# jimmc414/semantic_merge

Hardware: AMD Instinct MI355X
Metric: op-log compose+conflict throughput (ops/s), 100M-op logs, 1/2/4/8 GPUs (higher is better)
Workload: dtype u64; 1 GPU; c3: one merge of 100,000,000 ops (100,000,000 per GPU), 1,000,000 symbols, 64 ops/ms, seed 11; n_ops_per_gpu=100000000, n_ops_total=100000000, n_sym=1000000, composed_ops=99989720, conflicts=5140, plan=presorted, parallelism=single GPU

## Files before the change

semantic_merge_amd/csrc/smx_compose.hip:

```cpp
#include <algorithm>
#include <atomic>
#include <cstring>
#include <mutex>
#include <string>
#include <vector>

#include "smx_sort.h"
#include "smx_window.h"
#include "smx_small.h"
#include "smx_tables.h"


#include "smx_prof.h"

#include "smx_plan.h"
#include "smx_walk.h"

#include "smx_emit.h"


struct Layout {
  size_t off[64];
  size_t total;
};
// ... 341 lines not shown
      *out = g_side[i];
      return SMX_OK;
    }
  if (g_nside == SIDE_MAX) return SMX_OK;
  SideStream* S = new SideStream;
  S->dev = dev;
  S->caller = caller;
  int ncu = 0;
  HIP_TRY(hipDeviceGetAttribute(&ncu, hipDeviceAttributeMultiprocessorCount, dev));
  const int k = knob("SMX_SIDE_CUS", 0);
  if (k > 0 && k < ncu) {
    std::vector<uint32_t> mask((size_t)(ncu + 31) / 32, 0u);
    for (int i = 0; i < k; ++i) mask[(size_t)i / 32] |= 1u << (i % 32);
    HIP_TRY(hipExtStreamCreateWithCUMask(&S->s, (uint32_t)mask.size(), mask.data()));
  } else {
    HIP_TRY(hipStreamCreateWithFlags(&S->s, hipStreamNonBlocking));
  }
  const unsigned evf = hipEventDisableTiming | hipEventDisableSystemFence;
  HIP_TRY(hipEventCreateWithFlags(&S->fork, evf));
  HIP_TRY(hipEventCreateWithFlags(&S->join, evf));
  g_side[g_nside++] = S;
  *out = S;
  return SMX_OK;
}

#ifndef SMX_TB_UNSKIP_MAXN
#define SMX_TB_UNSKIP_MAXN (1 << 22)
#endif
#ifndef SMX_TB_OVERLAP_MIN
#define SMX_TB_OVERLAP_MIN (1 << 18)
#endif

static int launch_tail(const Ctx& C) {
  u64 width, nbk;
  const bool geo = tb_geometry(C, &width, &nbk);
  SideStream* S = nullptr;
  if (geo && C.n >= SMX_TB_OVERLAP_MIN && !knob("SMX_TB_SERIAL", 0)) {
    int rc = side_stream(C.st, &S);
    if (rc) return rc;
  }
  std::unique_lock<std::mutex> own;
  int rc;
  hipStream_t st = C.st;
  TbArgs A{};
  u32* lst = C.ws<u32>(B_TBHIST);
  u32* rec = C.ws<u32>(B_REC);
  if (S) {
    own = std::unique_lock<std::mutex>(S->mu);
    A = tb_args(C);
    A.width = (u32)width;
    A.nbk = (u32)nbk;
    A.keep_skip = C.n <= SMX_TB_UNSKIP_MAXN ? 2u : 1u;
    const int nblk = (int)SMX_CEIL_DIV((u64)C.n, (u64)TB_TILE);
    HIP_TRY(hipEventRecord(S->fork, st));
    HIP_TRY(hipStreamWaitEvent(S->s, S->fork, 0));
    hipLaunchKernelGGL(k_tb_scatter, dim3(nblk), dim3(TB_NT), 0, S->s, A, lst, rec);
    HIP_TRY(hipGetLastError());
    HIP_TRY(hipEventRecord(S->join, S->s));
  }
  C.tm->begin(ST_WALK);
  if ((rc = launch_walk(C, nullptr))) {
    if (S) (void)hipStreamWaitEvent(st, S->join, 0);
    return rc;
  }
  C.tm->end(ST_WALK);
  if (S) HIP_TRY(hipStreamWaitEvent(st, S->join, 0));
  C.tm->begin(ST_TABLES);
  bool bucketed = true;
  if (S) {
    if (A.keep_skip == 1u)
      hipLaunchKernelGGL(k_tb_unskip, dim3(1024), dim3(BLOCK), 0, st, A, lst, rec, C.ws<u32>(B_SKIPLIST));
    hipLaunchKernelGGL(k_tb_reduce, dim3(nbk), dim3(TBR_NT), 0, st, A, lst, rec, C.n_sym, C.ws<int4>(B_FIN),
                       PartTab{nullptr, 0u, 0, nullptr});
    HIP_TRY(hipGetLastError());
  } else if ((rc = launch_tables(C, nullptr, 0, 0, &bucketed))) {
    return rc;
  }
  C.tm->end(ST_TABLES);
  C.tm->begin(ST_EMIT);
  if ((rc = launch_emit(C, bucketed, nullptr))) return rc;
  C.tm->end(ST_EMIT);
  return SMX_OK;
}


struct EarlyFail {
  u32* flag_host = nullptr;
  u32* flag_dev = nullptr;
  hipEvent_t ev = nullptr;
};
enum WinLevel { WL_NORMAL, WL_WIDE };
static i64 level_cap(int lv) { return lv == WL_WIDE ? WF_WIDE_CAP : WF_CAP; }
static int first_level(const Ctx& C) { return knob("SMX_FIRST_WIDE", 0) ? WL_WIDE : WL_NORMAL; }
static i64 first_tgt(const Ctx& C) {
  return knob("SMX_WIN_TGT", first_level(C) == WL_WIDE ? WF_WIDE_CAP : WIN_TGT);
}

template <int CAP, int NT, bool DBG, bool MAP>
static void launch_window_f(const WinArgs& P, hipStream_t st) {
  hipLaunchKernelGGL((k_window_f<CAP, NT, DBG, MAP>), dim3(P.W), dim3(NT), 0, st, P);
}
template <int CAP, int NT>
static void launch_window_level(const WinArgs& P, hipStream_t st) {
  if (P.src_map) launch_window_f<CAP, NT, false, true>(P, st);
  else launch_window_f<CAP, NT, false, false>(P, st);
}

static int launch_presorted_windows(const Ctx& C, i64 W, i64 CM, int level) {
  const bool wide = level == WL_WIDE;
  hipStream_t st = C.st;
  WinArgs P = win_args(C);
  P.cpre = C.ws<u32>(B_CCNT);
  P.CM = CM;
  P.kts = C.ops->ts;
  P.khi = C.ops->oid_hi;
  P.klo = C.ops->oid_lo;
  P.perm = nullptr;
  P.W = W;
  P.ablate = knob("SMX_ABLATE", 0);
  const int stage = wide ? ST_WINDOW_WIDE : ST_WINDOW;
  C.tm->begin(stage);
#if SMX_DIAG
  if (g_phase_dbg && !P.src_map && (size_t)W * WF_NSTAMP * 8 <= g_phase_dbg_bytes) {
    P.dbg = (u64*)g_phase_dbg;
    if (wide) launch_window_f<WF_WIDE_CAP, WF_WIDE_NT, true, false>(P, st);
    else launch_window_f<WF_CAP, WF_NT, true, false>(P, st);
  } else
#endif
  if (wide) launch_window_level<WF_WIDE_CAP, WF_WIDE_NT>(P, st);
  else launch_window_level<WF_CAP, WF_NT>(P, st);
  HIP_TRY(hipGetLastError());
  C.tm->end(stage);
  return SMX_OK;
}

struct Deferred {
  bool on = false;
  i64 W = 0, W_w = 0, CM = 0;
};

struct PreGeo {
  i64 tgt, W, D, CM;
  u64 *sA, *sB;
};
static PreGeo presorted_geometry(const Ctx& C, i64 tgt, int level) {
  const i64 cap = level_cap(level);
  tgt = std::min(std::max(tgt, (i64)WIN_TGT_MIN), cap);
  tgt -= tgt % CH;
  u64* sA = C.ws<u64>(B_SMP);
  return PreGeo{tgt, SMX_CEIL_DIV(C.n, tgt), cap / CH, SMX_CEIL_DIV(std::max(C.na, C.nb), (i64)CH) + 1, sA,
                sA + SMX_CEIL_DIV(C.na, (i64)CH) + 1};
}

static int run_presorted(const Ctx& C, i64 tgt, const EarlyFail* early = nullptr, int level = WL_NORMAL,
                         Deferred* defer = nullptr) {
  hipStream_t st = C.st;
  ComposeMeta* meta = C.ws<ComposeMeta>(B_META);
  i64* bnd = C.ws<i64>(B_BND);
  C.tm->begin(ST_PLAN);
  static_assert(sizeof(ComposeMeta) % 4 == 0, "meta is zeroed by words");
  const PreGeo G = presorted_geometry(C, tgt, level);
  const i64 W = G.W, CM = G.CM;
  const bool cs_small = CM <= CS_SMALL_CM;
  {
    const int rc = zero_async(meta, sizeof(ComposeMeta), st);
    if (rc) return rc;
  }
  const i64 nchunk = SMX_CEIL_DIV(C.na, (i64)CH) + SMX_CEIL_DIV(C.nb, (i64)CH);
  u32* ccnt = C.ws<u32>(B_CCNT);
  const bool lmode = early && defer && level == WL_NORMAL;
  LongW lw{};
  if (lmode) {
    const PreGeo Gw = presorted_geometry(C, level_cap(WL_WIDE), WL_WIDE);
    lw.tgt_w = Gw.tgt;
    lw.W_w = Gw.W;
    lw.D_w = Gw.D;
  }
  hipLaunchKernelGGL(k_khist, dim3(SMX_CEIL_DIV(nchunk, (i64)CH_PER_BLOCK * KH_R)), dim3(KH_NT), 0, st,
                     C.ops->kind, C.ops->ts, C.na, C.nb, C.ops->b_gap, CM, ccnt, G.sA, G.sB, meta,
                     early ? early->flag_dev : nullptr, lmode ? G.D : (i64)0);
  if (lmode) HIP_TRY(hipEventRecord(early->ev, st));
  const i64 nfp = SMX_CEIL_DIV(W + 1, (i64)BLOCK);
  const bool fused = cs_small && !early;
  if (fused)
    hipLaunchKernelGGL(k_fpart_cscan, dim3(nfp + 2 * SMX_N_KINDS), dim3(BLOCK), 0, st, C.ops->ts,
                       C.ops->ts + C.na + C.ops->b_gap, G.sA, G.sB, C.na, C.nb, W, G.tgt, G.D, bnd, meta,
                       (u32*)nullptr, ccnt, CM, nfp);
  else
    hipLaunchKernelGGL(k_fpart, dim3(nfp), dim3(BLOCK), 0, st, C.ops->ts, C.ops->ts + C.na + C.ops->b_gap, G.sA,
                       G.sB, C.na, C.nb, W, G.tgt, G.D, bnd, meta, (early && !lmode) ? early->flag_dev : nullptr, lw);
  if (early && !lmode) HIP_TRY(hipEventRecord(early->ev, st));
  const u64 nwin_long = lmode ? (u64)lw.W_w : 0ull;
  if (fused) {
  } else if (cs_small) {
    hipLaunchKernelGGL(k_cscan_small, dim3(2 * SMX_N_KINDS), dim3(BLOCK), 0, st, ccnt, C.na, C.nb, CM, meta, (u64)W,
                       nwin_long);
  } else {
    const i64 NT = SMX_CEIL_DIV(CM, (i64)CS_TILE);
    u32* tsum = C.ws<u32>(B_TSUM);
    hipLaunchKernelGGL(k_cscan_up, dim3(NT, 2 * SMX_N_KINDS), dim3(BLOCK), 0, st, ccnt, C.na, C.nb, CM, NT, tsum,
                       meta);
    hipLaunchKernelGGL(k_cscan_mid, dim3(2 * SMX_N_KINDS), dim3(BLOCK), 0, st, tsum, C.na, C.nb, CM, NT, ccnt,
                       meta, (u64)W, nwin_long);
    hipLaunchKernelGGL(k_cscan_down, dim3(NT, 2 * SMX_N_KINDS), dim3(BLOCK), 0, st, ccnt, C.na, C.nb, CM, NT,
                       tsum, meta);
  }
  HIP_TRY(hipGetLastError());
  C.tm->end(ST_PLAN);
  if (lmode) {
    *defer = Deferred{true, W, lw.W_w, CM};
    return SMX_OK;
  }
  return launch_presorted_windows(C, W, CM, level);
}

__global__ void k_plan_rearm(ComposeMeta* meta, u64 nwin) {
  if (meta->f_fail == F_LONG) meta->f_fail = 0;
  meta->n_win = nwin;
}
static int run_presorted_rewide(const Ctx& C, i64 tgt, int level = WL_WIDE) {
  hipStream_t st = C.st;
  ComposeMeta* meta = C.ws<ComposeMeta>(B_META);
  const PreGeo G = presorted_geometry(C, tgt, level);
  C.tm->begin(ST_PLAN);
  hipLaunchKernelGGL(k_plan_rearm, dim3(1), dim3(1), 0, st, meta, (u64)G.W);
  hipLaunchKernelGGL(k_fpart, dim3(SMX_CEIL_DIV(G.W + 1, (i64)BLOCK)), dim3(BLOCK), 0, st, C.ops->ts,
                     C.ops->ts + C.na + C.ops->b_gap, G.sA, G.sB, C.na, C.nb, G.W, G.tgt, G.D, C.ws<i64>(B_BND), meta,
                     (u32*)nullptr, LongW{});
  HIP_TRY(hipGetLastError());
  C.tm->end(ST_PLAN);
  return launch_presorted_windows(C, G.W, G.CM, level);
}

#include "smx_segsort.h"

static hipError_t stream_wait(hipStream_t st) { return hipStreamSynchronize(st); }

static int run_generic(const Ctx& C, int mode) {
  hipStream_t st = C.st;
  ComposeMeta* meta = C.ws<ComposeMeta>(B_META);
  i64* bnd = C.ws<i64>(B_BND);
  u32* wcnt = C.ws<u32>(B_WCNT);
  u32* woff = C.ws<u32>(B_WOFF);
  const i64 na = C.na, nb = C.nb, n = C.n;
  u64* sts = C.ws<u64>(B_STS);
  u64* shi = C.ws<u64>(B_SHI);
  u64* slo = C.ws<u64>(B_SLO);
  u32* perm = C.ws<u32>(B_PERM);
  C.tm->begin(ST_GSORT);
  HIP_TRY(hipMemsetAsync(meta, 0, sizeof(ComposeMeta), st));
  if (mode == GEN_SEG) {
    C.tm->begin(ST_SEGSORT);
    for (int side = 0; side < 2; ++side) {
      const i64 off = side ? na : 0, cnt = side ? nb : na;
      if (cnt == 0) continue;
      hipLaunchKernelGGL(k_segsort, dim3(SMX_CEIL_DIV(cnt, (i64)SEG_H)), dim3(SEG_NT), 0, st, C.ops->ts + off,
                         C.ops->oid_hi + off, C.ops->oid_lo + off, cnt, (u32)off, sts + off, shi + off, slo + off,
                         perm + off, meta);
    }
    C.tm->end(ST_SEGSORT);
  } else {
    const bool with_lo = mode == GEN_RADIX_LO;
    hipLaunchKernelGGL(k_meta_init, dim3(1), dim3(1), 0, st, meta);
    hipLaunchKernelGGL(k_keymask, dim3(grid_for(n, BLOCK * 8)), dim3(BLOCK), 0, st, C.ops->ts, C.ops->oid_hi,
                       C.ops->oid_lo, na, n, meta);
    ComposeMeta hm;
    HIP_TRY(hipMemcpyAsync(&hm, meta, sizeof(ComposeMeta), hipMemcpyDeviceToHost, st));
    HIP_TRY(hipStreamSynchronize(st));
    RadixTemp rt{C.ws<u64>(B_RK2), C.ws<u32>(B_RV2), C.ws<u32>(B_RHIST), C.ws<u32>(B_PART)};
    const u64* words[3] = {C.ops->oid_lo, C.ops->oid_hi, C.ops->ts};
    const int w0 = with_lo ? 0 : 1;
    for (int side = 0; side < 2; ++side) {
      const i64 off = side ? na : 0, cnt = side ? nb : na;
      if (cnt == 0) continue;
      u64* key = C.ws<u64>(B_RKEY) + off;
      u32* val = perm + off;
      for (int wi = w0; wi < 3; ++wi) {
        const int q = 2 - wi;
        const u64 varying = hm.key_or[side][q] ^ hm.key_and[side][q];
        int shifts[8], ns = 0;
        for (int dgt = 0; dgt < 8; ++dgt)
          if ((varying >> (8 * dgt)) & 0xffull) shifts[ns++] = 8 * dgt;
        if (wi == w0) {
          hipLaunchKernelGGL(k_gather_init, dim3(grid_for(cnt)), dim3(BLOCK), 0, st, words[wi] + off, key, val,
                             cnt);
          if (off)
            hipLaunchKernelGGL(k_offset, dim3(grid_for(cnt)), dim3(BLOCK), 0, st, val, cnt, (u32)off);
        } else {
          hipLaunchKernelGGL(k_gather, dim3(grid_for(cnt)), dim3(BLOCK), 0, st, words[wi], val, key, cnt);
        }
        if (ns) HIP_TRY(radix_sort_pairs(key, val, cnt, shifts, ns, rt, st));
      }
      HIP_TRY(hipMemcpyAsync(sts + off, key, (size_t)cnt * 8, hipMemcpyDeviceToDevice, st));
      hipLaunchKernelGGL(k_gather2, dim3(grid_for(cnt)), dim3(BLOCK), 0, st, C.ops->oid_hi, C.ops->oid_lo, val,
                         shi + off, slo + off, cnt);
    }
    if (!with_lo) hipLaunchKernelGGL(k_dupcheck, dim3(grid_for(n)), dim3(BLOCK), 0, st, sts, shi, na, n, meta);
  }
  const i64 W = SMX_CEIL_DIV(n, (i64)WG_CAP);
  hipLaunchKernelGGL(k_gpart, dim3(SMX_CEIL_DIV(W + 1, (i64)BLOCK)), dim3(BLOCK), 0, st, sts, shi, slo, na, nb,
                     W, bnd, meta);
  hipLaunchKernelGGL(k_wcount, dim3(W), dim3(WC_NT), 0, st, C.ops->kind, C.ops->v0, C.ops->v1, perm, bnd, na, W,
                     wcnt, meta);
  hipLaunchKernelGGL(k_wscan, dim3(NCNT), dim3(BLOCK), 0, st, wcnt, woff, W, meta);
  hipLaunchKernelGGL(k_bases, dim3(1), dim3(1), 0, st, meta, (u64)W);
  HIP_TRY(hipGetLastError());
  C.tm->end(ST_GSORT);
  WinArgs P = win_args(C);
  P.kts = sts;
  P.khi = shi;
  P.klo = slo;
  P.perm = perm;
  P.W = W;
  P.ablate = 0;
  C.tm->begin(ST_WINDOW_G);
  hipLaunchKernelGGL(k_window_g, dim3(W), dim3(WG_NT), 0, st, P);
  HIP_TRY(hipGetLastError());
  C.tm->end(ST_WINDOW_G);
  return SMX_OK;
}

struct PinnedMeta {
  ComposeMeta* p = nullptr;
  ~PinnedMeta() {
    if (p) (void)hipHostFree(p);
  }
};
static int read_meta(const Ctx& C, ComposeMeta* hm) {
  static thread_local PinnedMeta holder;
  ComposeMeta*& pinned = holder.p;
  if (!pinned) HIP_TRY(hipHostMalloc((void**)&pinned, sizeof(ComposeMeta), hipHostMallocDefault));
  HIP_TRY(hipMemcpyAsync(pinned, C.ws<ComposeMeta>(B_META), sizeof(ComposeMeta), hipMemcpyDeviceToHost, C.st));
// ... 386 lines not shown
```

semantic_merge_amd/csrc/smx_plan.h:

```cpp
#pragma once

__global__ void __launch_bounds__(BLOCK) k_keymask(const u64* __restrict__ ts, const u64* __restrict__ hi,
                                                   const u64* __restrict__ lo, i64 na, i64 n,
                                                   ComposeMeta* meta) {
  u64 ro[2][3] = {{0, 0, 0}, {0, 0, 0}};
  u64 ra[2][3] = {{~0ull, ~0ull, ~0ull}, {~0ull, ~0ull, ~0ull}};
  for (i64 i = (i64)blockIdx.x * BLOCK + threadIdx.x; i < n; i += (i64)gridDim.x * BLOCK) {
    const u64 v[3] = {ts[i], hi[i], lo[i]};
    const int s = i >= na;
#pragma unroll
    for (int q = 0; q < 3; ++q) {
      ro[s][q] |= v[q];
      ra[s][q] &= v[q];
    }
  }
  __shared__ u32 sm[24];
  if (threadIdx.x < 24) sm[threadIdx.x] = 0;
  __syncthreads();
#pragma unroll
  for (int s = 0; s < 2; ++s)
#pragma unroll
    for (int q = 0; q < 3; ++q) {
      const u64 w[2] = {ro[s][q], ~ra[s][q]};
#pragma unroll
// ... 2 lines not shown
        if ((threadIdx.x & (WAVE - 1)) == WAVE - 1) {
          atomicOr(&sm[(s * 3 + q) * 4 + 2 * x], lo32);
          atomicOr(&sm[(s * 3 + q) * 4 + 2 * x + 1], hi32);
        }
      }
    }
  __syncthreads();
  if (threadIdx.x < 6) {
    const int s = threadIdx.x / 3, q = threadIdx.x % 3;
    const u32* v = &sm[threadIdx.x * 4];
    atomicOr((unsigned long long*)&meta->key_or[s][q], ((unsigned long long)v[1] << 32) | v[0]);
    atomicAnd((unsigned long long*)&meta->key_and[s][q], ~(((unsigned long long)v[3] << 32) | v[2]));
  }
}

__global__ void k_zero(u32* __restrict__ p, u64 nw) {
  for (u64 i = (u64)blockIdx.x * blockDim.x + threadIdx.x; i < nw; i += (u64)gridDim.x * blockDim.x) p[i] = 0u;
}
static int zero_async(void* p, size_t bytes, hipStream_t st) {
  if (bytes % 4) return set_err(SMX_E_ARG, "zero_async: size not a multiple of 4");
  const u64 nw = bytes / 4;
  if (nw == 0) return SMX_OK;
  u64 g = SMX_CEIL_DIV(nw, (u64)BLOCK * 4);
  if (g > 4096) g = 4096;
  hipLaunchKernelGGL(k_zero, dim3((u32)g), dim3(BLOCK), 0, st, (u32*)p, nw);
  HIP_TRY(hipGetLastError());
  return SMX_OK;
}

__global__ void k_meta_init(ComposeMeta* meta) {
  for (int s = 0; s < 2; ++s)
    for (int q = 0; q < 3; ++q) meta->key_and[s][q] = ~0ull;
}

struct LongW {
  i64 tgt_w = 0, W_w = 0, D_w = 0;
};
__device__ __forceinline__ void fpart_body(const u64* __restrict__ ts, const u64* __restrict__ tsB,
                                           const u64* __restrict__ sA, const u64* __restrict__ sB, i64 na, i64 nb,
                                           i64 W, i64 tgt, i64 D, i64* __restrict__ bnd, ComposeMeta* meta,
                                           u32* long_host, i64 blk, i64 nblk, LongW lw = LongW{}) {
  const i64 k = blk * BLOCK + threadIdx.x;
  bool chk = true;
  u64 fl = F_LONG;
  if (lw.tgt_w) {
    if ((__hip_atomic_load(&meta->f_fail, __ATOMIC_RELAXED, __HIP_MEMORY_SCOPE_AGENT) & F_LONG) == F_LONG) {
      W = lw.W_w, tgt = lw.tgt_w, D = lw.D_w;
      fl = F_WLONG;
      long_host = nullptr;
    } else {
      chk = false;
    }
  }
  if (chk) {
    const i64 nt = nblk * BLOCK, ca = SMX_CEIL_DIV(na, (i64)CH), cb = nb / CH;
    bool lg = false;
    for (i64 c = k; c + D < ca; c += nt) lg |= sA[c] == sA[c + D];
    for (i64 c = k; c + D < cb; c += nt) lg |= sB[c] == sB[c + D];
    const u64 lgw = __ballot(lg);
    if (lgw && (threadIdx.x & (WAVE - 1)) == 0 &&
        (__hip_atomic_load(&meta->f_fail, __ATOMIC_RELAXED, __HIP_MEMORY_SCOPE_AGENT) & fl) != fl) {
      atomicOr((unsigned long long*)&meta->f_fail, fl);
      if (long_host) __hip_atomic_store(long_host, 1u, __ATOMIC_RELAXED, __HIP_MEMORY_SCOPE_SYSTEM);
    }
    if (lgw) {
      if (k <= W) bnd[2 * k] = bnd[2 * k + 1] = 0;
      return;
    }
  }
  if (k > W) return;
  const i64 n = na + nb;
  const u64* A = ts;
  const u64* B = tsB;
  const i64 d = k * tgt;
  if (k == 0 || d >= n || k == W) {
    bnd[2 * k] = k == 0 ? 0 : na;
    bnd[2 * k + 1] = k == 0 ? 0 : nb;
    return;
  }
  const i64 lo0 = d - nb > 0 ? d - nb : 0, hi0 = d < na ? d : na;
  i64 lo = lo0, hi = hi0;
  if (lo < hi) {
    const i64 ilo = SMX_CEIL_DIV(lo, (i64)CH), ihi = (hi - 1) / CH;
    if (ilo <= ihi) {
      const i64 dj = d / CH - 1;
      i64 l = ilo, h = ihi + 1;
      while (l < h) {
        const i64 mid = (l + h) >> 1;
        if (sA[mid] <= sB[dj - mid]) l = mid + 1;
        else h = mid;
      }
      if (l > ilo) lo = CH * (l - 1) + 1;
      if (l <= ihi) hi = CH * l;
    }
    while (lo < hi) {
      const i64 mid = (lo + hi) >> 1;
      if (A[mid] <= B[d - 1 - mid]) lo = mid + 1;
      else hi = mid;
    }
  }
  const i64 a = lo, b = d - lo;
  const u64 tau = (a < na && (b >= nb || A[a] <= B[b])) ? A[a] : B[b];
  i64 r[2];
#pragma unroll
  for (int s = 0; s < 2; ++s) {
    const u64* X = s ? B : A;
    i64 h = s ? b : a;
    i64 step = 1, l = 0;
    while (h > 0) {
      const i64 cand = h - step > 0 ? h - step : 0;
      if (X[cand] < tau) {
        l = cand + 1;
        break;
      }
      h = cand;
      step *= 2;
    }
    while (l < h) {
      const i64 mid = (l + h) >> 1;
      if (X[mid] < tau) l = mid + 1;
      else h = mid;
    }
    r[s] = l;
  }
  bnd[2 * k] = r[0];
  bnd[2 * k + 1] = r[1];
}
__global__ void k_fpart(const u64* __restrict__ ts, const u64* __restrict__ tsB, const u64* __restrict__ sA,
                        const u64* __restrict__ sB, i64 na, i64 nb, i64 W, i64 tgt, i64 D, i64* __restrict__ bnd,
                        ComposeMeta* meta, u32* long_host, LongW lw) {
  fpart_body(ts, tsB, sA, sB, na, nb, W, tgt, D, bnd, meta, long_host, blockIdx.x, gridDim.x, lw);
}

__global__ void k_gpart(const u64* __restrict__ sts, const u64* __restrict__ shi,
                        const u64* __restrict__ slo, i64 na, i64 nb, i64 W, i64* __restrict__ bnd,
                        const ComposeMeta* meta) {
  const i64 k = (i64)blockIdx.x * BLOCK + threadIdx.x;
  if (k > W || meta->f_fail) return;
  const i64 n = na + nb;
  const i64 d = k * WG_CAP;
  if (k == 0) { bnd[0] = 0; bnd[1] = 0; return; }
  if (d >= n || k == W) { bnd[2 * k] = na; bnd[2 * k + 1] = nb; return; }
  i64 lo = d - nb > 0 ? d - nb : 0, hi = d < na ? d : na;
  while (lo < hi) {
    i64 mid = (lo + hi) >> 1;
    const i64 j = na + d - 1 - mid;
    if (key_le(sts[mid], shi[mid], slo[mid], sts[j], shi[j], slo[j])) lo = mid + 1;
    else hi = mid;
  }
  bnd[2 * k] = lo;
  bnd[2 * k + 1] = d - lo;
}

#ifndef KH_NT
#define KH_NT 512
#endif
#define CH_PER_BLOCK (KH_NT / 16)
#ifndef KH_R
#define KH_R 1
#endif

__global__ void __launch_bounds__(KH_NT) k_khist(const u8* __restrict__ kind, const u64* __restrict__ ts,
                                                 i64 na, i64 nb, i64 bgap, i64 CM, u32* __restrict__ cnt,
                                                 u64* __restrict__ sA, u64* __restrict__ sB, ComposeMeta* meta,
                                                 u32* long_host, i64 Dl) {
  __shared__ u32 c[CH_PER_BLOCK * KH_R][SMX_N_KINDS];
  __shared__ u32 km[2];
  __shared__ u32 lgb;
  const i64 CA = SMX_CEIL_DIV(na, (i64)CH), CB = SMX_CEIL_DIV(nb, (i64)CH);
  const int j = threadIdx.x / 16, q = threadIdx.x % 16;
  if (threadIdx.x < 2) km[threadIdx.x] = 0;
  if (threadIdx.x == 0) lgb = 0;
  u32 w[KH_R][4];
  int nvr[KH_R];
  u64 smpA[KH_R], smpB[KH_R], farA[KH_R], farB[KH_R];
  u64* atA[KH_R];
  u64* atB[KH_R];
  bool chkA[KH_R], chkB[KH_R];
#pragma unroll
  for (int rd = 0; rd < KH_R; ++rd) {
    const i64 g = ((i64)blockIdx.x * KH_R + rd) * CH_PER_BLOCK + j;
    const int side = g >= CA;
    const i64 cc = side ? g - CA : g;
    const i64 len = side ? nb : na;
    const i64 r0 = cc * CH + q * 16;
    const int nv = g < CA + CB ? (int)(len - r0 < 0 ? 0 : (len - r0 < 16 ? len - r0 : 16)) : 0;
    nvr[rd] = nv;
    const u8* src = kind + (side ? na + bgap : 0) + r0;
    w[rd][0] = w[rd][1] = w[rd][2] = w[rd][3] = 0u;
    if (nv == 16 && (reinterpret_cast<uintptr_t>(src) & 15) == 0) {
      const uint4 v = *reinterpret_cast<const uint4*>(src);
      w[rd][0] = v.x; w[rd][1] = v.y; w[rd][2] = v.z; w[rd][3] = v.w;
    } else {
#pragma unroll
      for (int y = 0; y < 16; ++y)
        if (y < nv) w[rd][y >> 2] |= (u32)src[y] << (8 * (y & 3));
    }
    atA[rd] = atB[rd] = nullptr;
    smpA[rd] = smpB[rd] = farA[rd] = farB[rd] = 0;
    chkA[rd] = chkB[rd] = false;
    if (g < CA + CB) {
      if (!side && q == 0) {
        atA[rd] = sA + cc;
        smpA[rd] = ts[cc * CH];
        if (Dl > 0 && cc + Dl < CA) {
          chkA[rd] = true;
          farA[rd] = ts[(cc + Dl) * CH];
        }
      }
      if (side && q == 15 && nv == 16) {
        atB[rd] = sB + cc;
        smpB[rd] = ts[na + bgap + cc * CH + CH - 1];
        if (Dl > 0 && cc + Dl < nb / CH) {
          chkB[rd] = true;
          farB[rd] = ts[na + bgap + (cc + Dl) * CH + CH - 1];
        }
      }
    }
  }
  bool bad = false;
#pragma unroll
  for (int rd = 0; rd < KH_R; ++rd) {
    const int nv = nvr[rd];
    u32 pk[3] = {0u, 0u, 0u};
#pragma unroll
    for (int y = 0; y < 16; ++y) {
      if (y >= nv) break;
      u32 k = (w[rd][y >> 2] >> (8 * (y & 3))) & 0xffu;
      bad |= k >= SMX_N_KINDS;
      k = k < SMX_N_KINDS ? k : SMX_N_KINDS - 1;
      const u32 wd = (k * 43u) >> 8;
      const u32 inc = 1u << (5u * (k - 6u * wd));
      pk[0] += wd == 0 ? inc : 0u;
      pk[1] += wd == 1 ? inc : 0u;
      pk[2] += wd == 2 ? inc : 0u;
    }
    u32 f[6];
#pragma unroll
    for (int i = 0; i < 3; ++i) {
      f[2 * i] = (pk[i] & 31u) | ((pk[i] >> 5) & 31u) << 10 | ((pk[i] >> 10) & 31u) << 20;
      f[2 * i + 1] = ((pk[i] >> 15) & 31u) | ((pk[i] >> 20) & 31u) << 10 | ((pk[i] >> 25) & 31u) << 20;
    }
#pragma unroll
    for (int i = 0; i < 6; ++i) {
      u32 v = f[i];
      v += dpp_u32<0x111, 0xf>(v);
      v += dpp_u32<0x112, 0xf>(v);
      v += dpp_u32<0x114, 0xf>(v);
      v += dpp_u32<0x118, 0xf>(v);
      f[i] = v;
    }
    if (q == 15) {
#pragma unroll
      for (int k = 0; k < SMX_N_KINDS; ++k) c[rd * CH_PER_BLOCK + j][k] = (f[k / 3] >> (10 * (k % 3))) & 1023u;
    }
  }
  bool lg = false;
#pragma unroll
  for (int rd = 0; rd < KH_R; ++rd) {
    if (atA[rd]) *atA[rd] = smpA[rd];
    if (atB[rd]) *atB[rd] = smpB[rd];
    lg |= (chkA[rd] && farA[rd] == smpA[rd]) || (chkB[rd] && farB[rd] == smpB[rd]);
  }
  if (__ballot(lg) && (threadIdx.x & (WAVE - 1)) == 0) atomicOr(&lgb, 1u);
  if (__ballot(bad) && (threadIdx.x & (WAVE - 1)) == 0) {
    meta->bad_sym = 1;
    if (long_host) __hip_atomic_store(long_host + 1, 1u, __ATOMIC_RELAXED, __HIP_MEMORY_SCOPE_SYSTEM);
  }
  __syncthreads();
  if (threadIdx.x == 0 && lgb &&
      (__hip_atomic_load(&meta->f_fail, __ATOMIC_RELAXED, __HIP_MEMORY_SCOPE_AGENT) & F_LONG) != F_LONG) {
    const u64 was = atomicOr((unsigned long long*)&meta->f_fail, F_LONG);
    if ((was & F_LONG) != F_LONG && long_host)
      __hip_atomic_store(long_host, 1u, __ATOMIC_RELAXED, __HIP_MEMORY_SCOPE_SYSTEM);
  }
  u32 m0 = 0, m1 = 0;
  for (int i = threadIdx.x; i < CH_PER_BLOCK * KH_R * SMX_N_KINDS; i += KH_NT) {
    const int jj = i % (CH_PER_BLOCK * KH_R), k = i / (CH_PER_BLOCK * KH_R);
    const i64 gg = (i64)blockIdx.x * CH_PER_BLOCK * KH_R + jj;
    if (gg >= CA + CB) continue;
    const int sd = gg >= CA;
    const u32 v = c[jj][k];
    cnt[((i64)sd * SMX_N_KINDS + k) * CM + (sd ? gg - CA : gg)] = v;
    if (v) (sd ? m1 : m0) |= 1u << k;
  }
  m0 = wave_or_to_last(m0);
  m1 = wave_or_to_last(m1);
  if ((threadIdx.x & (WAVE - 1)) == WAVE - 1) {
    if (m0) atomicOr(&km[0], m0);
    if (m1) atomicOr(&km[1], m1);
  }
  __syncthreads();
  if (threadIdx.x < 2 && km[threadIdx.x]) {
    const u32 cur = __hip_atomic_load(&meta->kmask[threadIdx.x], __ATOMIC_RELAXED, __HIP_MEMORY_SCOPE_AGENT);
    if ((cur | km[threadIdx.x]) != cur) atomicOr(&meta->kmask[threadIdx.x], km[threadIdx.x]);
  }
}

__device__ __forceinline__ bool cs_present(const ComposeMeta* meta, int col) {
  return (meta->kmask[col >= SMX_N_KINDS] >> (col % SMX_N_KINDS)) & 1u;
}

#define CS_TILE (BLOCK * 8)

__global__ void __launch_bounds__(BLOCK) k_cscan_up(const u32* __restrict__ cnt, i64 na, i64 nb, i64 CM,
                                                    i64 NT, u32* __restrict__ tsum, const ComposeMeta* meta) {
  __shared__ u32 s[NWAVES + 1];
  const int col = blockIdx.y;
  if (!cs_present(meta, col)) return;
  const i64 C = SMX_CEIL_DIV(col >= SMX_N_KINDS ? nb : na, (i64)CH);
  const i64 t0 = (i64)blockIdx.x * CS_TILE;
  if (t0 >= C) return;
  const u32* colp = cnt + (i64)col * CM;
  const i64 b = t0 + (i64)threadIdx.x * 8;
  u32 acc = 0;
#pragma unroll
  for (int j = 0; j < 8; ++j) acc += b + j < C ? colp[b + j] : 0u;
  u32 tot;
  block_excl_scan<OpSum, u32>(acc, s, &tot);
  if (threadIdx.x == 0) tsum[(i64)col * NT + blockIdx.x] = tot;
}

__device__ __forceinline__ void set_n_win(ComposeMeta* meta, u64 nwin, u64 nwin_long) {
  if (nwin_long && meta->f_fail == F_LONG) {
    meta->f_fail = 0;
    nwin = nwin_long;
  }
  meta->n_win = nwin;
}

__global__ void __launch_bounds__(BLOCK) k_cscan_mid(u32* __restrict__ tsum, i64 na, i64 nb, i64 CM, i64 NT,
                                                     u32* __restrict__ cnt, ComposeMeta* meta, u64 nwin,
                                                     u64 nwin_long) {
  __shared__ u32 s[NWAVES + 1];
  const int col = blockIdx.x;
  const int side = col / SMX_N_KINDS, k = col % SMX_N_KINDS;
  const i64 C = SMX_CEIL_DIV(side ? nb : na, (i64)CH);
  const i64 nt = cs_present(meta, col) ? SMX_CEIL_DIV(C, (i64)CS_TILE) : 0;
  u32 carry = 0;
  for (i64 r0 = 0; r0 < nt; r0 += BLOCK) {
    const i64 r = r0 + threadIdx.x;
    const u32 v = r < nt ? tsum[(i64)col * NT + r] : 0u;
    u32 tot;
    const u32 ex = block_excl_scan<OpSum, u32>(v, s, &tot);
    if (r < nt) tsum[(i64)col * NT + r] = carry + ex;
    carry += tot;
  }
  if (threadIdx.x == 0) {
    cnt[(i64)col * CM + C] = carry;
    atomicAdd((unsigned long long*)&meta->kcnt[k], (unsigned long long)carry);
    if (k == KREN) meta->n_ren_side[side] = carry;
    __threadfence();
    if (atomicAdd((unsigned long long*)&meta->cs_done, 1ull) == (unsigned long long)gridDim.x - 1) {
      __threadfence();
      set_n_win(meta, nwin, nwin_long);
      u64 acc = 0;
      for (int kk = 0; kk < SMX_N_KINDS; ++kk) {
        meta->base[kk] = acc;
        acc += __hip_atomic_load(&meta->kcnt[kk], __ATOMIC_RELAXED, __HIP_MEMORY_SCOPE_AGENT);
      }
      meta->base[SMX_N_KINDS] = acc;
    }
  }
}

__global__ void __launch_bounds__(BLOCK) k_cscan_down(u32* __restrict__ cnt, i64 na, i64 nb, i64 CM, i64 NT,
                                                      const u32* __restrict__ tsum, const ComposeMeta* meta) {
  __shared__ u32 s[NWAVES + 1];
  const int col = blockIdx.y;
  if (!cs_present(meta, col)) return;
  const i64 C = SMX_CEIL_DIV(col >= SMX_N_KINDS ? nb : na, (i64)CH);
  const i64 t0 = (i64)blockIdx.x * CS_TILE;
  if (t0 >= C) return;
  u32* colp = cnt + (i64)col * CM;
  const i64 b = t0 + (i64)threadIdx.x * 8;
  u32 v[8];
  u32 acc = 0;
#pragma unroll
  for (int j = 0; j < 8; ++j) {
    v[j] = b + j < C ? colp[b + j] : 0u;
    acc += v[j];
  }
  u32 tot;
  u32 run = tsum[(i64)col * NT + blockIdx.x] + block_excl_scan<OpSum, u32>(acc, s, &tot);
#pragma unroll
  for (int j = 0; j < 8; ++j) {
    if (b + j < C) colp[b + j] = run;
    run += v[j];
  }
}

#ifndef CS_SMALL_CM
#define CS_SMALL_CM 16384
#endif
__device__ __forceinline__ void cscan_small_body(u32* __restrict__ cnt, i64 na, i64 nb, i64 CM, ComposeMeta* meta,
                                                 u64 nwin, int col, u32* s, u64 nwin_long = 0) {
  const int side = col / SMX_N_KINDS, k = col % SMX_N_KINDS;
  const i64 C = SMX_CEIL_DIV(side ? nb : na, (i64)CH);
  u32* colp = cnt + (i64)col * CM;
  u32 carry = 0;
  if (cs_present(meta, col)) {
    for (i64 t0 = 0; t0 < C; t0 += CS_TILE) {
      const i64 b = t0 + (i64)threadIdx.x * 8;
      u32 v[8];
      u32 acc = 0;
#pragma unroll
      for (int j = 0; j < 8; ++j) {
        v[j] = b + j < C ? colp[b + j] : 0u;
        acc += v[j];
      }
      u32 tot;
      u32 run = carry + block_excl_scan<OpSum, u32>(acc, s, &tot);
#pragma unroll
      for (int j = 0; j < 8; ++j) {
        if (b + j < C) colp[b + j] = run;
        run += v[j];
      }
      carry += tot;
    }
  }
  if (threadIdx.x == 0) {
    colp[C] = carry;
    atomicAdd((unsigned long long*)&meta->kcnt[k], (unsigned long long)carry);
    if (k == KREN) meta->n_ren_side[side] = carry;
    __threadfence();
    if (atomicAdd((unsigned long long*)&meta->cs_done, 1ull) == (unsigned long long)(2 * SMX_N_KINDS - 1)) {
      __threadfence();
      set_n_win(meta, nwin, nwin_long);
      u64 acc = 0;
      for (int kk = 0; kk < SMX_N_KINDS; ++kk) {
        meta->base[kk] = acc;
        acc += __hip_atomic_load(&meta->kcnt[kk], __ATOMIC_RELAXED, __HIP_MEMORY_SCOPE_AGENT);
      }
      meta->base[SMX_N_KINDS] = acc;
    }
  }
}
__global__ void __launch_bounds__(BLOCK) k_cscan_small(u32* __restrict__ cnt, i64 na, i64 nb, i64 CM,
                                                       ComposeMeta* meta, u64 nwin, u64 nwin_long) {
  __shared__ u32 s[NWAVES + 1];
  cscan_small_body(cnt, na, nb, CM, meta, nwin, blockIdx.x, s, nwin_long);
}
__global__ void __launch_bounds__(BLOCK) k_fpart_cscan(const u64* __restrict__ ts, const u64* __restrict__ tsB,
                                                       const u64* __restrict__ sA, const u64* __restrict__ sB, i64 na,
                                                       i64 nb, i64 W, i64 tgt, i64 D, i64* __restrict__ bnd,
                                                       ComposeMeta* meta, u32* long_host, u32* __restrict__ cnt,
                                                       i64 CM, i64 nfp) {
  __shared__ u32 s[NWAVES + 1];
// ... 180 lines not shown
```

Before: 43.57 billion ops/s.

## Make k_khist persistent with per-wave tiles, prefetch and SWAR kind counting

Rewrites the kind histogram kernel as a persistent grid sized to CUs times four workgroups. Each wave processes 32-chunk tiles and double-buffers the next tile's loads. Kind counts use a branch-light SWAR bit-shift accumulation in place of a per-byte compare chain, and per-wave LDS staging with wave-local syncs replaces block-wide barriers. Sampling and long-window checks now use lane shuffles. The aim is to cut launch and tail overhead and raise memory-level parallelism on this bandwidth-bound pass, at the cost of more complex packing code and the risk of field overflow or occupancy loss.

```diff
diff --git a/semantic_merge_amd/csrc/smx_compose.hip b/semantic_merge_amd/csrc/smx_compose.hip
--- a/semantic_merge_amd/csrc/smx_compose.hip
+++ b/semantic_merge_amd/csrc/smx_compose.hip
@@ -517,6 +517,21 @@
                 sA + SMX_CEIL_DIV(C.na, (i64)CH) + 1};
 }
 
+static int device_cus(int* cus) {
+  constexpr int DEV_MAX = 64;
+  static std::atomic<int> known[DEV_MAX];
+  int dev = 0;
+  HIP_TRY(hipGetDevice(&dev));
+  int n = dev >= 0 && dev < DEV_MAX ? known[dev].load(std::memory_order_relaxed) : 0;
+  if (n <= 0) {
+    HIP_TRY(hipDeviceGetAttribute(&n, hipDeviceAttributeMultiprocessorCount, dev));
+    if (n <= 0) return set_err(SMX_E_HIP, "device reports no compute units");
+    if (dev >= 0 && dev < DEV_MAX) known[dev].store(n, std::memory_order_relaxed);
+  }
+  *cus = n;
+  return SMX_OK;
+}
+
 static int run_presorted(const Ctx& C, i64 tgt, const EarlyFail* early = nullptr, int level = WL_NORMAL,
                          Deferred* defer = nullptr) {
   hipStream_t st = C.st;
@@ -541,8 +556,14 @@
     lw.W_w = Gw.W;
     lw.D_w = Gw.D;
   }
-  hipLaunchKernelGGL(k_khist, dim3(SMX_CEIL_DIV(nchunk, (i64)CH_PER_BLOCK * KH_R)), dim3(KH_NT), 0, st,
-                     C.ops->kind, C.ops->ts, C.na, C.nb, C.ops->b_gap, CM, ccnt, G.sA, G.sB, meta,
+  int ncu = 0;
+  {
+    const int rc = device_cus(&ncu);
+    if (rc) return rc;
+  }
+  const i64 kh_grid = std::max<i64>(
+      1, std::min<i64>((i64)ncu * KH_WG_PER_CU, SMX_CEIL_DIV(SMX_CEIL_DIV(nchunk, (i64)KH_TILE), (i64)KH_NW)));
+  hipLaunchKernelGGL(k_khist, dim3((u32)kh_grid), dim3(KH_NT), 0, st, C.ops->kind, C.ops->ts, C.na, C.nb, C.ops->b_gap, CM, ccnt, G.sA, G.sB, meta,
                      early ? early->flag_dev : nullptr, lmode ? G.D : (i64)0);
   if (lmode) HIP_TRY(hipEventRecord(early->ev, st));
   const i64 nfp = SMX_CEIL_DIV(W + 1, (i64)BLOCK);
diff --git a/semantic_merge_amd/csrc/smx_plan.h b/semantic_merge_amd/csrc/smx_plan.h
--- a/semantic_merge_amd/csrc/smx_plan.h
+++ b/semantic_merge_amd/csrc/smx_plan.h
@@ -178,148 +178,211 @@
   bnd[2 * k + 1] = d - lo;
 }
 
-#ifndef KH_NT
-#define KH_NT 512
-#endif
-#define CH_PER_BLOCK (KH_NT / 16)
-#ifndef KH_R
-#define KH_R 1
-#endif
+#define KH_NT BLOCK
+#define KH_NW (KH_NT / WAVE)
+#define KH_WG_PER_CU 4
+#define KH_TILE 32
+#define KH_SUB (KH_TILE / 4)
+#define KH_PKW 8
+#define KH_PKS (KH_PKW + 1)
+#define KH_PAD ((u32)SMX_N_KINDS)
+
+struct KhTile {
+  uint4 w[KH_SUB];
+  u64 smp;
+  u32 fl;
+};
+
+__device__ __forceinline__ void kh_load(KhTile& T, i64 t, int lane, const u8* __restrict__ kind,
+                                        const u64* __restrict__ ts, i64 na, i64 nb, i64 bgap, i64 CA, i64 CB,
+                                        i64 Dl, bool& bad) {
+  const int q = lane & 15;
+  u32 fl = 0;
+#pragma unroll
+  for (int s = 0; s < KH_SUB; ++s) {
+    const i64 g = t * KH_TILE + s * 4 + (lane >> 4);
+    const int side = g >= CA;
+    const i64 cc = side ? g - CA : g;
+    const i64 r0 = cc * CH + q * 16;
+    const i64 left = g < CA + CB ? (side ? nb : na) - r0 : 0;
+    const u8* src = kind + (side ? na + bgap : 0) + r0;
+    if (left >= 16 && (reinterpret_cast<uintptr_t>(src) & 15) == 0) {
+      T.w[s] = *reinterpret_cast<const uint4*>(src);
+      fl |= 1u << s;
+    } else {
+      u64 d[2] = {0x0101010101010101ull * KH_PAD, 0x0101010101010101ull * KH_PAD};
+      const int nv = left < 0 ? 0 : (left < 16 ? (int)left : 16);
+      for (int y = 0; y < nv; ++y) {
+        u32 k = src[y];
+        bad |= k >= SMX_N_KINDS;
+        k = k < SMX_N_KINDS ? k : SMX_N_KINDS - 1;
+        const u64 x = (u64)(k ^ KH_PAD) << (8 * (y & 7));
+        d[0] ^= y < 8 ? x : 0ull;
+        d[1] ^= y < 8 ? 0ull : x;
+      }
+      T.w[s] = make_uint4((u32)d[0], (u32)(d[0] >> 32), (u32)d[1], (u32)(d[1] >> 32));
+    }
+  }
+  {
+    const bool far = lane >= 32;
+    const i64 g = t * KH_TILE + (lane & 31);
+    const int side = g >= CA;
+    const i64 cf = (side ? g - CA : g) + (far ? Dl : 0);
+    const bool ok = g < CA + CB && cf < (side ? nb / CH : CA) && (!far || Dl > 0);
+    T.smp = 0;
+    if (ok) {
+      T.smp = side ? ts[na + bgap + cf * CH + CH - 1] : ts[cf * CH];
+      fl |= 256u;
+    }
+  }
+  T.fl = fl;
+}
+
+__device__ __forceinline__ u32 kh_word(u32 i) { return i < 5 ? (i & 1u) : 2u + ((i - 5u) & 1u); }
+__device__ __forceinline__ u32 kh_shift(u32 i) { return 12u * ((i < 5 ? i : i - 5u) >> 1); }
+constexpr u64 kh_fields(int width, int period, int n) {
+  u64 m = 0;
+  for (int i = 0; i < n; ++i) m |= ((1ull << width) - 1) << (i * period);
+  return m;
+}
+__device__ __forceinline__ void kh_count(u32 (&w)[4], bool unchecked, bool& bad, u32 (&f)[KH_PKW]) {
+  u32 h = 0;
+#pragma unroll
+  for (int i = 0; i < 4; ++i) h |= ((w[i] & 0x7f7f7f7fu) + 0x6e6e6e6eu) | w[i];
+  const bool bw = unchecked && (h & 0x80808080u);
+  if (__ballot(bw)) {
+    bad |= bw;
+    if (bw) {
+#pragma unroll
+      for (int i = 0; i < 4; ++i) {
+        u32 x = 0;
+#pragma unroll
+        for (int b = 0; b < 4; ++b) {
+          const u32 k = (w[i] >> (8 * b)) & 0xffu;
+          x |= (k < SMX_N_KINDS ? k : SMX_N_KINDS - 1) << (8 * b);
+        }
+        w[i] = x;
+      }
+    }
+  }
+  u64 a[3] = {0, 0, 0};
+#pragma unroll
+  for (int i = 0; i < 4; ++i) {
+    const u32 w3 = w[i] + (w[i] << 1);
+#pragma unroll
+    for (int b = 0; b < 4; ++b) {
+      const int y = 4 * i + b;
+      a[y < 7 ? 0 : (y < 14 ? 1 : 2)] += 1ull << ((w3 >> (8 * b)) & 0xffu);
+    }
+  }
+  constexpr u64 ME = kh_fields(3, 6, 9);
+  const u64 eo[2] = {(a[0] & ME) + (a[1] & ME) + (a[2] & ME),
+                     ((a[0] >> 3) & ME) + ((a[1] >> 3) & ME) + ((a[2] >> 3) & ME)};
+#pragma unroll
+  for (int p = 0; p < 2; ++p) {
+    const u32 lo = (u32)eo[p], hi = (u32)(eo[p] >> 30);
+    f[4 * p + 0] = lo & 0x3f03f03fu;
+    f[4 * p + 1] = (lo >> 6) & 0x0003f03fu;
+    f[4 * p + 2] = hi & 0x0003f03fu;
+    f[4 * p + 3] = (hi >> 6) & 0x0003f03fu;
+  }
+#pragma unroll
+  for (int i = 0; i < KH_PKW; ++i) {
+    u32 v = f[i];
+    v += dpp_u32<0x111, 0xf>(v);
+    v += dpp_u32<0x112, 0xf>(v);
+    v += dpp_u32<0x114, 0xf>(v);
+    v += dpp_u32<0x118, 0xf>(v);
+    f[i] = v;
+  }
+}
 
 __global__ void __launch_bounds__(KH_NT) k_khist(const u8* __restrict__ kind, const u64* __restrict__ ts,
                                                  i64 na, i64 nb, i64 bgap, i64 CM, u32* __restrict__ cnt,
                                                  u64* __restrict__ sA, u64* __restrict__ sB, ComposeMeta* meta,
                                                  u32* long_host, i64 Dl) {
-  __shared__ u32 c[CH_PER_BLOCK * KH_R][SMX_N_KINDS];
-  __shared__ u32 km[2];
-  __shared__ u32 lgb;
+  __shared__ u32 pk[KH_NW][KH_TILE][KH_PKS];
+  __shared__ u32 red[KH_NW][4];
   const i64 CA = SMX_CEIL_DIV(na, (i64)CH), CB = SMX_CEIL_DIV(nb, (i64)CH);
-  const int j = threadIdx.x / 16, q = threadIdx.x % 16;
-  if (threadIdx.x < 2) km[threadIdx.x] = 0;
-  if (threadIdx.x == 0) lgb = 0;
-  u32 w[KH_R][4];
-  int nvr[KH_R];
-  u64 smpA[KH_R], smpB[KH_R], farA[KH_R], farB[KH_R];
-  u64* atA[KH_R];
-  u64* atB[KH_R];
-  bool chkA[KH_R], chkB[KH_R];
-#pragma unroll
-  for (int rd = 0; rd < KH_R; ++rd) {
-    const i64 g = ((i64)blockIdx.x * KH_R + rd) * CH_PER_BLOCK + j;
-    const int side = g >= CA;
-    const i64 cc = side ? g - CA : g;
-    const i64 len = side ? nb : na;
-    const i64 r0 = cc * CH + q * 16;
-    const int nv = g < CA + CB ? (int)(len - r0 < 0 ? 0 : (len - r0 < 16 ? len - r0 : 16)) : 0;
-    nvr[rd] = nv;
-    const u8* src = kind + (side ? na + bgap : 0) + r0;
-    w[rd][0] = w[rd][1] = w[rd][2] = w[rd][3] = 0u;
-    if (nv == 16 && (reinterpret_cast<uintptr_t>(src) & 15) == 0) {
-      const uint4 v = *reinterpret_cast<const uint4*>(src);
-      w[rd][0] = v.x; w[rd][1] = v.y; w[rd][2] = v.z; w[rd][3] = v.w;
-    } else {
-#pragma unroll
-      for (int y = 0; y < 16; ++y)
-        if (y < nv) w[rd][y >> 2] |= (u32)src[y] << (8 * (y & 3));
-    }
-    atA[rd] = atB[rd] = nullptr;
-    smpA[rd] = smpB[rd] = farA[rd] = farB[rd] = 0;
-    chkA[rd] = chkB[rd] = false;
-    if (g < CA + CB) {
-      if (!side && q == 0) {
-        atA[rd] = sA + cc;
-        smpA[rd] = ts[cc * CH];
-        if (Dl > 0 && cc + Dl < CA) {
-          chkA[rd] = true;
-          farA[rd] = ts[(cc + Dl) * CH];
-        }
-      }
-      if (side && q == 15 && nv == 16) {
-        atB[rd] = sB + cc;
-        smpB[rd] = ts[na + bgap + cc * CH + CH - 1];
-        if (Dl > 0 && cc + Dl < nb / CH) {
-          chkB[rd] = true;
-          farB[rd] = ts[na + bgap + (cc + Dl) * CH + CH - 1];
-        }
-      }
-    }
-  }
-  bool bad = false;
-#pragma unroll
-  for (int rd = 0; rd < KH_R; ++rd) {
-    const int nv = nvr[rd];
-    u32 pk[3] = {0u, 0u, 0u};
-#pragma unroll
-    for (int y = 0; y < 16; ++y) {
-      if (y >= nv) break;
-      u32 k = (w[rd][y >> 2] >> (8 * (y & 3))) & 0xffu;
-      bad |= k >= SMX_N_KINDS;
-      k = k < SMX_N_KINDS ? k : SMX_N_KINDS - 1;
-      const u32 wd = (k * 43u) >> 8;
-      const u32 inc = 1u << (5u * (k - 6u * wd));
-      pk[0] += wd == 0 ? inc : 0u;
-      pk[1] += wd == 1 ? inc : 0u;
-      pk[2] += wd == 2 ? inc : 0u;
-    }
-    u32 f[6];
-#pragma unroll
-    for (int i = 0; i < 3; ++i) {
-      f[2 * i] = (pk[i] & 31u) | ((pk[i] >> 5) & 31u) << 10 | ((pk[i] >> 10) & 31u) << 20;
-      f[2 * i + 1] = ((pk[i] >> 15) & 31u) | ((pk[i] >> 20) & 31u) << 10 | ((pk[i] >> 25) & 31u) << 20;
-    }
-#pragma unroll
-    for (int i = 0; i < 6; ++i) {
-      u32 v = f[i];
-      v += dpp_u32<0x111, 0xf>(v);
-      v += dpp_u32<0x112, 0xf>(v);
-      v += dpp_u32<0x114, 0xf>(v);
-      v += dpp_u32<0x118, 0xf>(v);
-      f[i] = v;
-    }
-    if (q == 15) {
-#pragma unroll
-      for (int k = 0; k < SMX_N_KINDS; ++k) c[rd * CH_PER_BLOCK + j][k] = (f[k / 3] >> (10 * (k % 3))) & 1023u;
-    }
-  }
-  bool lg = false;
-#pragma unroll
-  for (int rd = 0; rd < KH_R; ++rd) {
-    if (atA[rd]) *atA[rd] = smpA[rd];
-    if (atB[rd]) *atB[rd] = smpB[rd];
-    lg |= (chkA[rd] && farA[rd] == smpA[rd]) || (chkB[rd] && farB[rd] == smpB[rd]);
-  }
-  if (__ballot(lg) && (threadIdx.x & (WAVE - 1)) == 0) atomicOr(&lgb, 1u);
-  if (__ballot(bad) && (threadIdx.x & (WAVE - 1)) == 0) {
-    meta->bad_sym = 1;
-    if (long_host) __hip_atomic_store(long_host + 1, 1u, __ATOMIC_RELAXED, __HIP_MEMORY_SCOPE_SYSTEM);
-  }
-  __syncthreads();
-  if (threadIdx.x == 0 && lgb &&
-      (__hip_atomic_load(&meta->f_fail, __ATOMIC_RELAXED, __HIP_MEMORY_SCOPE_AGENT) & F_LONG) != F_LONG) {
-    const u64 was = atomicOr((unsigned long long*)&meta->f_fail, F_LONG);
-    if ((was & F_LONG) != F_LONG && long_host)
-      __hip_atomic_store(long_host, 1u, __ATOMIC_RELAXED, __HIP_MEMORY_SCOPE_SYSTEM);
-  }
+  const int lane = threadIdx.x & (WAVE - 1);
+  const int wv = __builtin_amdgcn_readfirstlane(threadIdx.x / WAVE);
+  const i64 ntile = SMX_CEIL_DIV(CA + CB, (i64)KH_TILE);
+  const i64 per = SMX_CEIL_DIV(ntile, (i64)gridDim.x);
+  const i64 t1 = ((i64)blockIdx.x + 1) * per < ntile ? ((i64)blockIdx.x + 1) * per : ntile;
+  bool bad = false, lg = false;
   u32 m0 = 0, m1 = 0;
-  for (int i = threadIdx.x; i < CH_PER_BLOCK * KH_R * SMX_N_KINDS; i += KH_NT) {
-    const int jj = i % (CH_PER_BLOCK * KH_R), k = i / (CH_PER_BLOCK * KH_R);
-    const i64 gg = (i64)blockIdx.x * CH_PER_BLOCK * KH_R + jj;
-    if (gg >= CA + CB) continue;
-    const int sd = gg >= CA;
-    const u32 v = c[jj][k];
-    cnt[((i64)sd * SMX_N_KINDS + k) * CM + (sd ? gg - CA : gg)] = v;
-    if (v) (sd ? m1 : m0) |= 1u << k;
-  }
+  KhTile cur, nxt;
+  i64 t = (i64)blockIdx.x * per + wv;
+  if (t < t1) kh_load(cur, t, lane, kind, ts, na, nb, bgap, CA, CB, Dl, bad);
+  for (; t < t1; t += KH_NW) {
+    const bool more = t + KH_NW < t1;
+    if (more) kh_load(nxt, t + KH_NW, lane, kind, ts, na, nb, bgap, CA, CB, Dl, bad);
+#pragma unroll
+    for (int s = 0; s < KH_SUB; ++s) {
+      u32 w[4] = {cur.w[s].x, cur.w[s].y, cur.w[s].z, cur.w[s].w};
+      u32 f[KH_PKW];
+      kh_count(w, (cur.fl >> s) & 1u, bad, f);
+      if ((lane & 15) == 15) {
+#pragma unroll
+        for (int i = 0; i < KH_PKW; ++i) pk[wv][4 * s + (lane >> 4)][i] = f[i];
+      }
+    }
+    {
+      const i64 g = t * KH_TILE + (lane & 31);
+      const bool have = (cur.fl >> 8) & 1u;
+      const u64 far = __shfl_down(cur.smp, 32, WAVE);
+      const bool fhave = __shfl_down((int)have, 32, WAVE);
+      if (lane < 32 && have) {
+        if (g >= CA) sB[g - CA] = cur.smp;
+        else sA[g] = cur.smp;
+        lg |= fhave && far == cur.smp;
+      }
+    }
+    wave_lds_sync();
+#pragma unroll
+    for (int i = 0; i < KH_TILE * SMX_N_KINDS / WAVE; ++i) {
+      const u32 idx = (u32)(i * WAVE + lane), k = idx / KH_TILE, jj = idx % KH_TILE;
+      const i64 gg = t * KH_TILE + jj;
+      const u32 v = (pk[wv][jj][4 * (k & 1u) + kh_word(k >> 1)] >> kh_shift(k >> 1)) & 0xfffu;
+      if (gg < CA + CB) {
+        const int sd = gg >= CA;
+        cnt[((i64)sd * SMX_N_KINDS + k) * CM + (sd ? gg - CA : gg)] = v;
+        if (v) (sd ? m1 : m0) |= 1u << k;
+      }
+    }
+    wave_lds_sync();
+    if (more) cur = nxt;
+  }
+  static_assert(KH_TILE * SMX_N_KINDS % WAVE == 0, "the flush takes whole waves");
   m0 = wave_or_to_last(m0);
   m1 = wave_or_to_last(m1);
-  if ((threadIdx.x & (WAVE - 1)) == WAVE - 1) {
-    if (m0) atomicOr(&km[0], m0);
-    if (m1) atomicOr(&km[1], m1);
+  const bool lgw = __ballot(lg) != 0, badw = __ballot(bad) != 0;
+  if (lane == WAVE - 1) {
+    red[wv][0] = m0;
+    red[wv][1] = m1;
+    red[wv][2] = lgw;
+    red[wv][3] = badw;
   }
   __syncthreads();
-  if (threadIdx.x < 2 && km[threadIdx.x]) {
-    const u32 cur = __hip_atomic_load(&meta->kmask[threadIdx.x], __ATOMIC_RELAXED, __HIP_MEMORY_SCOPE_AGENT);
-    if ((cur | km[threadIdx.x]) != cur) atomicOr(&meta->kmask[threadIdx.x], km[threadIdx.x]);
+  if (threadIdx.x < 4) {
+    u32 r = 0;
+#pragma unroll
+    for (int i = 0; i < KH_NW; ++i) r |= red[i][threadIdx.x];
+    if (threadIdx.x < 2) {
+      if (r) {
+        const u32 have = __hip_atomic_load(&meta->kmask[threadIdx.x], __ATOMIC_RELAXED, __HIP_MEMORY_SCOPE_AGENT);
+        if ((have | r) != have) atomicOr(&meta->kmask[threadIdx.x], r);
+      }
+    } else if (threadIdx.x == 2) {
+      if (r && (__hip_atomic_load(&meta->f_fail, __ATOMIC_RELAXED, __HIP_MEMORY_SCOPE_AGENT) & F_LONG) != F_LONG) {
+        const u64 was = atomicOr((unsigned long long*)&meta->f_fail, F_LONG);
+        if ((was & F_LONG) != F_LONG && long_host)
+          __hip_atomic_store(long_host, 1u, __ATOMIC_RELAXED, __HIP_MEMORY_SCOPE_SYSTEM);
+      }
+    } else if (r) {
+      meta->bad_sym = 1;
+      if (long_host) __hip_atomic_store(long_host + 1, 1u, __ATOMIC_RELAXED, __HIP_MEMORY_SCOPE_SYSTEM);
+    }
   }
 }
 
```

Measured after the change: 43.96 billion ops/s (median of 6 runs). About the same (+0.9%).
